# regicide211212/multi-style-transfer-gan

Measured on AMD Instinct MI355X. Metric: train-step images/sec (fwd+bwd+loss), 256x256 batch32, higher is better.
Workload: dtype f32; 1 GPU; config 3: reference CycleGAN train_step (2x EnhancedGenerator + 2x EnhancedDiscriminator, channels=16, num_transformer_blocks=0), 32 image pairs/GPU at 256x256, fwd+bwd+loss+Adam; per_gpu_batch=32, size=256, channels=16, parallelism=dp1, collective=none, losses_finite=True

## Files before the change

### multi-style-transfer-gan_amd/mstg_hip/csrc/common.h

```cpp
#pragma once
#include <hip/hip_runtime.h>
#include <stdint.h>
#include <stdio.h>
#include <string.h>

#include "mstg_hip.h"

typedef float f32x4 __attribute__((ext_vector_type(4)));
typedef float f32x2 __attribute__((ext_vector_type(2)));

namespace mstg {

extern thread_local char g_last_error[256];
inline int fail_launch(hipError_t e, const char* what) {
    snprintf(g_last_error, sizeof(g_last_error), "%s: %s", what, hipGetErrorString(e));
    return MSTG_E_LAUNCH;
}
inline int fail_arg(int code, const char* what) {
    snprintf(g_last_error, sizeof(g_last_error), "%s", what);
    return code;
}
#define MSTG_CHECK_LAUNCH(what)                                   \
    do {                                                          \
        hipError_t e__ = hipGetLastError();                       \
        if (e__ != hipSuccess) return mstg::fail_launch(e__, what); \
    } while (0)

extern bool g_prof_on;
void prof_begin(const void* host_fn, hipStream_t st);
void prof_end(hipStream_t st);
#define MSTG_LAUNCH(kern, grid, block, lds, st, ...)                               \
    do {                                                                           \
        const bool prof__ = mstg::g_prof_on;                                       \
        if (prof__) mstg::prof_begin((const void*)(kern), (hipStream_t)(st));      \
        hipLaunchKernelGGL(kern, grid, block, lds, st, __VA_ARGS__);               \
        if (prof__) mstg::prof_end((hipStream_t)(st));                             \
    } while (0)

extern thread_local bool t_ws_packed;
#define MSTG_PACK_LAUNCH(...)                      \
    do {                                           \
        if (!mstg::t_ws_packed) MSTG_LAUNCH(__VA_ARGS__); \
    } while (0)

enum EnvKnob {
    ENV_ATTN_BLK4, ENV_ATTN_BLK64, ENV_WGRAD_1X1, ENV_WGRAD_TS_MAXCH, ENV_WGRAD_PLAIN, ENV_WGRAD_OLD, ENV_NO_DPACK, ENV_IGEMM,
    ENV_STREAM, ENV_PF, ENV_WGLOB, ENV_HEAVY_PER_CU, ENV_DBG, ENV_DBG_LDS_KB, ENV_MS_WGRAD_PACKED, ENV_MS_FWD4, ENV_NO_PACK_CACHE,
    ENV_P32, ENV_P32_TH, ENV_P32_WLDS, ENV_P32_DBG, ENV_P32_OCC, ENV_ATTN_REG, ENV_NFW_ADAPT, ENV_BSUMS_ALL, ENV_ATTN_BIG32, ENV_NORM_WGS,
    ENV_CONV_IMG, ENV_COUNT
};
const char* env_get(EnvKnob k);

int cu_count();
struct OccCache {
    const void* kern = nullptr;
    size_t lds = 0;
    int occ = 1;
};
int persistent_occupancy(OccCache& c, const void* kern, size_t lds);

constexpr int WAVE = 64;

__device__ __forceinline__ f32x4 mfma16(float a, float b, f32x4 c) {
    return __builtin_amdgcn_mfma_f32_16x16x4f32(a, b, c, 0, 0, 0);
}

__device__ __forceinline__ float wave_sum(float v) {
#pragma unroll
    for (int o = 32; o > 0; o >>= 1) v += __shfl_xor(v, o, 64);
    return v;
}

__device__ __forceinline__ float apply_act(float v, int act) {
    switch (act) {
        case MSTG_ACT_RELU: return v > 0.f ? v : 0.f;
        case MSTG_ACT_LEAKY02: return v > 0.f ? v : 0.2f * v;
        case MSTG_ACT_TANH: return tanhf(v);
        case MSTG_ACT_GELU: return 0.5f * v * (1.f + erff(v * 0.70710678118654752f));
        default: return v;
    }
}
__device__ __forceinline__ float act_grad(float v, int act) {
    switch (act) {
        case MSTG_ACT_RELU: return v > 0.f ? 1.f : 0.f;
        case MSTG_ACT_LEAKY02: return v > 0.f ? 1.f : 0.2f;
        case MSTG_ACT_TANH: return 1.f - v * v;
        case MSTG_ACT_GELU: return 0.5f * (1.f + erff(v * 0.70710678118654752f)) + v * 0.3989422804014327f * expf(-0.5f * v * v);
        default: return 1.f;
    }
}

__device__ __forceinline__ int xcd_swizzle(int bid, int nblk) {
    const int q = nblk >> 3, r = nblk & 7, xcd = bid & 7, k = bid >> 3;
    return (xcd < r ? xcd * (q + 1) : r * (q + 1) + (xcd - r) * q) + k;
}


__host__ __device__ __forceinline__ unsigned magic_u32(unsigned d) { return 0xFFFFFFFFu / d + 1u; }

template <int NB>
__device__ __forceinline__ void stage_window_batch(const float* __restrict__ img, float* __restrict__ lds, int total, int e0, int cols,
                                                   int nq, unsigned m_cols, unsigned m_nq, int y0, int x0, int H, int W, int ctot,
                                                   int nq_valid, int ckp, int tid, int rowpad) {
    f32x4 v[NB];
    int dst[NB];
    bool ok[NB];
#pragma unroll
    for (int k = 0; k < NB; ++k) {
        const int e = e0 + 256 * k + tid;
        const int p = nq == 1 ? e : (int)__umulhi((unsigned)e, m_nq);
        const int q = e - p * nq;
        const int r = (int)__umulhi((unsigned)p, m_cols), c = p - r * cols;
        const int iy = y0 + r, ix = x0 + c;
        ok[k] = e < total && (unsigned)iy < (unsigned)H && (unsigned)ix < (unsigned)W && q < nq_valid;
        const unsigned off = ok[k] ? (unsigned)(iy * W + ix) * (unsigned)ctot + 4u * q : 0u;
        v[k] = *reinterpret_cast<const f32x4*>(img + off);
        dst[k] = e < total ? p * ckp + 4 * q + r * rowpad : -1;
    }
#pragma unroll
    for (int k = 0; k < NB; ++k)
        if (dst[k] >= 0) *reinterpret_cast<f32x4*>(&lds[dst[k]]) = ok[k] ? v[k] : f32x4{0.f, 0.f, 0.f, 0.f};
}

__device__ __forceinline__ void stage_window(const float* __restrict__ img, float* __restrict__ lds, int rows, int cols, int nq,
                                             unsigned m_cols, unsigned m_nq, int y0, int x0, int H, int W, int ctot, int nq_valid,
                                             int ckp, int tid, int rowpad = 0) {
    const int total = rows * cols * nq;
    int e0 = 0;
    for (; e0 + 1024 < total; e0 += 2048)
        stage_window_batch<8>(img, lds, total, e0, cols, nq, m_cols, m_nq, y0, x0, H, W, ctot, nq_valid, ckp, tid, rowpad);
    for (; e0 < total; e0 += 1024)
        stage_window_batch<4>(img, lds, total, e0, cols, nq, m_cols, m_nq, y0, x0, H, W, ctot, nq_valid, ckp, tid, rowpad);
// ... 38 lines not shown
```

### multi-style-transfer-gan_amd/mstg_hip/csrc/msblock.hip

```cpp
#include "common.h"
#include <stdlib.h>

namespace mstg {

constexpr int MS_TH = 8, MS_PH = MS_TH + 8, MS_PW = 16 + 8, MS_CKP = 20;

template <int CH>
__global__ __launch_bounds__(256) void wgrad_ms_kernel(const float* __restrict__ x, const float* __restrict__ dy,
                                                       float* __restrict__ partial, int N, int H, int W, int tiles_x, int tiles_y,
                                                       int ntiles) {
    constexpr int NFH = CH / 16, C4 = CH / 4, U = NFH + 24, UW = (U + 3) / 4, BNP = CH + 4, NG = CH / 16;
    constexpr int PSTRIDE = NG * U * 256 + CH;
    extern __shared__ __attribute__((aligned(16))) float smem[];
    float* patch = smem;
    float* ht = smem + MS_PH * MS_PW * MS_CKP;

    const int tid = threadIdx.x, lane = tid & 63, wave = tid >> 6, i = lane & 15, g = lane >> 4;
    const int gchunk = blockIdx.y, g0 = 16 * gchunk;

    f32x4 acc[UW];
    int toff[UW], hfo[UW];
#pragma unroll
    for (int k = 0; k < UW; ++k) {
        const int u = min(wave + 4 * k, U - 1);
        int dyp = 0, dxp = 0, frag = u;
        if (u >= NFH) {
            const int r = (u - NFH) >> 3, i8 = (u - NFH) & 7, t9 = i8 < 4 ? i8 : i8 + 1, d = 1 << r;
            dyp = (t9 / 3 - 1) * d;
            dxp = (t9 % 3 - 1) * d;
            frag = ((r + 1) * C4) / 16;
        }
        toff[k] = ((4 + dyp) * MS_PW + 4 + dxp) * MS_CKP;
        hfo[k] = 16 * frag;
        acc[k] = f32x4{0.f, 0.f, 0.f, 0.f};
    }
    const int nu = (U - wave + 3) / 4;

    const bool do_bias = gchunk == 0;
    float bsum = 0.f;
    const unsigned m_pw = magic_u32(MS_PW), m_nq = magic_u32(CH / 4);
    const size_t plane = (size_t)H * W;
    for (int tile = blockIdx.x; tile < ntiles; tile += gridDim.x) {
        const int tx0 = tile % tiles_x, ty0 = (tile / tiles_x) % tiles_y, n = tile / (tiles_x * tiles_y);
        __syncthreads();
        stage_window(x + (size_t)n * plane * CH + g0, patch, MS_PH, MS_PW, 4, m_pw, 0x40000000u, ty0 * MS_TH - 4, tx0 * 16 - 4, H, W, CH, 4,
                     MS_CKP, tid);
        stage_window(dy + (size_t)n * plane * CH, ht, MS_TH, 16, CH / 4, 0x10000000u, m_nq, ty0 * MS_TH, tx0 * 16, H, W, CH, CH / 4, BNP, tid);
        __syncthreads();
        if (do_bias && tid < CH) {
#pragma unroll 8
            for (int p = 0; p < MS_TH * 16; ++p) bsum += ht[p * BNP + tid];
        }
#pragma unroll 1
        for (int r = 0; r < MS_TH; ++r) {
#pragma unroll 2
            for (int xs = 0; xs < 4; ++xs) {
                const int c = 4 * xs + g;
                const int abase = (r * MS_PW + c) * MS_CKP + i;
                const int hbase = (r * 16 + c) * BNP + i;
                float af[UW], bf[UW];
#pragma unroll
                for (int k = 0; k < UW; ++k) { af[k] = patch[abase + toff[k]]; bf[k] = ht[hbase + hfo[k]]; }
#pragma unroll
                for (int k = 0; k < UW; ++k) acc[k] = mfma16(af[k], bf[k], acc[k]);
            }
        }
    }
    float* out = partial + (size_t)blockIdx.x * PSTRIDE;
    if (do_bias && tid < CH) out[NG * U * 256 + tid] = bsum;
#pragma unroll
    for (int k = 0; k < UW; ++k) {
        if (k >= nu) continue;
        const int u = wave + 4 * k;
        float* o = out + ((size_t)gchunk * U + u) * 256;
#pragma unroll
        for (int e = 0; e < 4; ++e) o[(4 * g + e) * 16 + i] = acc[k][e];
    }
}

template <int CH>
struct MsUnits {
    static constexpr int NFW = CH / 16, C4 = CH / 4, U = NFW + 24;
    __host__ __device__ static constexpr int ring(int u) { return (u - NFW) >> 3; }
    __host__ __device__ static constexpr int t9(int u) { return ((u - NFW) & 7) < 4 ? ((u - NFW) & 7) : ((u - NFW) & 7) + 1; }
    __host__ __device__ static constexpr int oy(int u) { return u < NFW ? 0 : (t9(u) / 3 - 1) * (1 << ring(u)); }
    __host__ __device__ static constexpr int ox(int u) { return u < NFW ? 0 : (t9(u) % 3 - 1) * (1 << ring(u)); }
    __host__ __device__ static constexpr int frag(int u) { return u < NFW ? u : ((ring(u) + 1) * C4) / 16; }
};

struct MsParamPtrs {
    const float* w[4];
    const float* b[4];
};

template <int CH>
__global__ void ms_pack_fwd_kernel(MsParamPtrs prm, float* __restrict__ wp) {
    typedef MsUnits<CH> G;
    constexpr int NCH = CH / 16, TOTAL = NCH * G::U * 256;
    for (int idx = blockIdx.x * blockDim.x + threadIdx.x; idx < TOTAL + CH; idx += gridDim.x * blockDim.x) {
        if (idx >= TOTAL) {
            const int co = idx - TOTAL;
            wp[idx] = prm.b[co / G::C4][co % G::C4];
            continue;
        }
        const int j = idx & 3, lane = (idx >> 2) & 63, u = (idx >> 8) % G::U, chunk = idx / (G::U * 256);
        const int i = lane & 15, g = lane >> 4, ci = 16 * chunk + 4 * g + j;
        float v = 0.f;
        if (u < G::NFW) {
            const int co = 16 * u + i, br = co / G::C4, cj = co % G::C4;
            v = br == 0 ? prm.w[0][cj * CH + ci] : prm.w[br][(cj * CH + ci) * 9 + 4];
        } else {
            const int r = (u - G::NFW) >> 3, i8 = (u - G::NFW) & 7, t9 = i8 < 4 ? i8 : i8 + 1, br = r + 1;
            const int co = 16 * ((br * G::C4) / 16) + i;
            if (co >= br * G::C4 && co < (br + 1) * G::C4) v = prm.w[br][((co - br * G::C4) * CH + ci) * 9 + t9];
        }
        wp[idx] = v;
    }
}

template <int CH, int UB, int UE>
struct MsFwdUnitLoop {
    template <typename ACC>
    static __device__ __forceinline__ void run(ACC& acc, const float* __restrict__ wpc, const float* __restrict__ patch, int pbase, int lane) {
        typedef MsUnits<CH> G;
        constexpr int u = UB;
        const f32x4 a = *reinterpret_cast<const f32x4*>(wpc + u * 256 + lane * 4);
        constexpr int off = (G::oy(u) * MS_PW + G::ox(u)) * MS_CKP;
        f32x4 b[2];
#pragma unroll
        for (int pf = 0; pf < 2; ++pf) b[pf] = *reinterpret_cast<const f32x4*>(&patch[pbase + pf * MS_PW * MS_CKP + off]);
#pragma unroll
        for (int j = 0; j < 4; ++j)
#pragma unroll
            for (int pf = 0; pf < 2; ++pf) acc[G::frag(u)][pf] = mfma16(a[j], b[pf][j], acc[G::frag(u)][pf]);
        MsFwdUnitLoop<CH, UB + 1, UE>::run(acc, wpc, patch, pbase, lane);
    }
};
template <int CH, int UE>
struct MsFwdUnitLoop<CH, UE, UE> {
    template <typename ACC>
    static __device__ __forceinline__ void run(ACC&, const float*, const float*, int, int) {}
};

template <int CH>
__global__ __launch_bounds__(256) void ms_fwd_kernel(const float* __restrict__ x, const float* __restrict__ wp, float* __restrict__ y,
                                                     int N, int H, int W, int tiles_x, int tiles_y) {
    typedef MsUnits<CH> G;
    constexpr int NFW = G::NFW, NCH = CH / 16, PF = 2;
    extern __shared__ __attribute__((aligned(16))) float smem[];
    float* patch = smem;
    const int tid = threadIdx.x, lane = tid & 63, wave = tid >> 6, i = lane & 15, g = lane >> 4;
    const int tile = xcd_swizzle(blockIdx.x, gridDim.x);
// ... 85 lines not shown
        for (int wf = 0; wf < NFW; ++wf) a[wf] = *reinterpret_cast<const f32x4*>(wpc + ((wf * K::NQ + Q) * 64 + lane) * 4);
#pragma unroll
        for (int e = 0; e < 4; ++e) {
            constexpr int s0 = 4 * Q;
            const int s = s0 + e;
            if (s < K::NS) {
                const int off = (K::oy(s) * MS_PW + K::ox(s)) * MS_CKP + 4 * K::grp(s);
                float b[2];
#pragma unroll
                for (int pf = 0; pf < 2; ++pf) b[pf] = patch[pbase + pf * MS_PW * MS_CKP + off];
#pragma unroll
                for (int wf = 0; wf < NFW; ++wf)
#pragma unroll
                    for (int pf = 0; pf < 2; ++pf) acc[wf][pf] = mfma16(a[wf][e], b[pf], acc[wf][pf]);
            }
        }
        MsDgQuadLoop<CH, C, QB + 1, QE>::run(acc, wpc, patch, pbase, lane);
    }
};
template <int CH, int C, int QE>
struct MsDgQuadLoop<CH, C, QE, QE> {
    template <typename ACC>
    static __device__ __forceinline__ void run(ACC&, const float*, const float*, int, int) {}
};

template <int CH, int C, typename ACC>
__device__ __forceinline__ void ms_dgrad_chunk(ACC& acc, const float* __restrict__ dy_img, const float* __restrict__ wp, float* patch,
                                               int ty0, int tx0, int H, int W, unsigned m_pw, int pbase, int tid, int lane) {
    typedef MsDgChunk<CH, C> K;
    constexpr int NFW = CH / 16;
    if (C) __syncthreads();
    stage_window(dy_img + 16 * C, patch, MS_PH, MS_PW, 4, m_pw, 0x40000000u, ty0 * MS_TH - 4, tx0 * 16 - 4, H, W, CH, 4, MS_CKP, tid);
    __syncthreads();
    MsDgQuadLoop<CH, C, 0, K::NQ>::run(acc, wp + (size_t)ms_dg_quads_before<CH>(C) * NFW * 256, patch, pbase, lane);
}

template <int CH>
__global__ __launch_bounds__(256) void ms_dgrad_kernel(const float* __restrict__ dy, const float* __restrict__ wp,
                                                       const float* __restrict__ dres, float* __restrict__ dx, int N, int H, int W,
                                                       int tiles_x, int tiles_y) {
    constexpr int NFW = CH / 16, PF = 2;
    extern __shared__ __attribute__((aligned(16))) float smem[];
    float* patch = smem;
    const int tid = threadIdx.x, lane = tid & 63, wave = tid >> 6, i = lane & 15, g = lane >> 4;
    const int tile = xcd_swizzle(blockIdx.x, gridDim.x);
    const int tx0 = tile % tiles_x, ty0 = (tile / tiles_x) % tiles_y, n = tile / (tiles_x * tiles_y);
    const size_t plane = (size_t)H * W;
    const unsigned m_pw = magic_u32(MS_PW);
    f32x4 acc[NFW][PF];
#pragma unroll
    for (int wf = 0; wf < NFW; ++wf)
#pragma unroll
        for (int pf = 0; pf < PF; ++pf) acc[wf][pf] = f32x4{0.f, 0.f, 0.f, 0.f};
    const int pbase = ((PF * wave + 4) * MS_PW + i + 4) * MS_CKP + g;
    const float* dy_img = dy + (size_t)n * plane * CH;
    ms_dgrad_chunk<CH, 0>(acc, dy_img, wp, patch, ty0, tx0, H, W, m_pw, pbase, tid, lane);
    if (CH >= 32) ms_dgrad_chunk<CH, (CH >= 32 ? 1 : 0)>(acc, dy_img, wp, patch, ty0, tx0, H, W, m_pw, pbase, tid, lane);
    if (CH >= 64) {
        ms_dgrad_chunk<CH, (CH >= 64 ? 2 : 0)>(acc, dy_img, wp, patch, ty0, tx0, H, W, m_pw, pbase, tid, lane);
        ms_dgrad_chunk<CH, (CH >= 64 ? 3 : 0)>(acc, dy_img, wp, patch, ty0, tx0, H, W, m_pw, pbase, tid, lane);
    }
#pragma unroll
    for (int pf = 0; pf < PF; ++pf) {
        const int gy = ty0 * MS_TH + PF * wave + pf, gx = tx0 * 16 + i;
        if (gy < H && gx < W) {
            const size_t o = (((size_t)n * H + gy) * W + gx) * CH + 4 * g;
#pragma unroll
            for (int wf = 0; wf < NFW; ++wf) {
                f32x4 v = acc[wf][pf];
                if (dres) v += *reinterpret_cast<const f32x4*>(dres + o + 16 * wf);
                *reinterpret_cast<f32x4*>(dx + o + 16 * wf) = v;
            }
        }
    }
}

template <int CH>
struct MsPk {
    static constexpr int NFH = CH / 16, C4 = CH / 4, TPU = 16 / C4, UPB = 8 / TPU, U = NFH + 3 * UPB, UW = (U + 3) / 4;
    static constexpr int NG = CH / 16, PSTRIDE = NG * U * 256 + CH, LDY = CH + 4;
};

template <int CH>
__global__ __launch_bounds__(256) void wgrad_msp_kernel(const float* __restrict__ x, const float* __restrict__ dy,
                                                        float* __restrict__ partial, int N, int H, int W, int tiles_x, int tiles_y,
                                                        int ntiles) {
    typedef MsPk<CH> G;
    constexpr int UW = G::UW, U = G::U, LDY = G::LDY, MG = G::NG, LDX = CH + 4;
    extern __shared__ __attribute__((aligned(16))) float smem[];
    float* xs = smem;
    float* dyp = smem + MS_TH * 16 * LDX;

    const int tid = threadIdx.x, lane = tid & 63, wave = tid >> 6, i = lane & 15, g = lane >> 4;

    f32x4 acc[UW][MG];
    int boff[UW];
#pragma unroll
    for (int k = 0; k < UW; ++k) {
        const int u = min(wave + 4 * k, U - 1);
        int off;
        if (u < G::NFH) {
            off = 16 * u + i;
        } else {
            const int j = 1 + (u - G::NFH) / G::UPB, m = (u - G::NFH) % G::UPB;
            const int sidx = i / G::C4, co = i % G::C4, i8 = m * G::TPU + sidx, t9 = i8 < 4 ? i8 : i8 + 1, d = 1 << (j - 1);
            const int oy = (t9 / 3 - 1) * d, ox = (t9 % 3 - 1) * d;
            off = (-oy * MS_PW - ox) * LDY + j * G::C4 + co;
        }
        boff[k] = off;
#pragma unroll
        for (int mf = 0; mf < MG; ++mf) acc[k][mf] = f32x4{0.f, 0.f, 0.f, 0.f};
    }
    const int nu = (U - wave + 3) / 4;

    float bsum = 0.f;
    const unsigned m_pw = magic_u32(MS_PW), m_nq = magic_u32(CH / 4);
    const size_t plane = (size_t)H * W;
    for (int tile = blockIdx.x; tile < ntiles; tile += gridDim.x) {
        const int tx0 = tile % tiles_x, ty0 = (tile / tiles_x) % tiles_y, n = tile / (tiles_x * tiles_y);
        __syncthreads();
        stage_window(x + (size_t)n * plane * CH, xs, MS_TH, 16, CH / 4, 0x10000000u, m_nq, ty0 * MS_TH, tx0 * 16, H, W, CH, CH / 4, LDX, tid);
        stage_window(dy + (size_t)n * plane * CH, dyp, MS_PH, MS_PW, CH / 4, m_pw, m_nq, ty0 * MS_TH - 4, tx0 * 16 - 4, H, W, CH, CH / 4, LDY,
                     tid);
        __syncthreads();
        if (tid < CH) {
            for (int r = 0; r < MS_TH; ++r)
#pragma unroll 8
                for (int c = 0; c < 16; ++c) bsum += dyp[((r + 4) * MS_PW + c + 4) * LDY + tid];
        }
#pragma unroll 1
        for (int r = 0; r < MS_TH; ++r) {
#pragma unroll 2
            for (int xs4 = 0; xs4 < 4; ++xs4) {
                const int c = 4 * xs4 + g;
                float af[MG], bf[UW];
#pragma unroll
                for (int mf = 0; mf < MG; ++mf) af[mf] = xs[(r * 16 + c) * LDX + 16 * mf + i];
                const int bbase = ((r + 4) * MS_PW + c + 4) * LDY;
#pragma unroll
                for (int k = 0; k < UW; ++k) bf[k] = dyp[bbase + boff[k]];
#pragma unroll
                for (int k = 0; k < UW; ++k)
#pragma unroll
                    for (int mf = 0; mf < MG; ++mf) acc[k][mf] = mfma16(af[mf], bf[k], acc[k][mf]);
            }
        }
    }
    float* out = partial + (size_t)blockIdx.x * G::PSTRIDE;
    if (tid < CH) out[G::NG * U * 256 + tid] = bsum;
#pragma unroll
    for (int k = 0; k < UW; ++k) {
        if (k >= nu) continue;
        const int u = wave + 4 * k;
#pragma unroll
        for (int mf = 0; mf < MG; ++mf) {
            float* o = out + ((size_t)mf * U + u) * 256;
#pragma unroll
            for (int e = 0; e < 4; ++e) o[(4 * g + e) * 16 + i] = acc[k][mf][e];
        }
    }
}

constexpr int M4_TH = 16, M4_PH = M4_TH + 8;

template <int CH, int JB, int T9, int Q>
struct Ms4Step {
    static constexpr int C4 = CH / 4, RS = C4 / 4;
    static __device__ __forceinline__ void run(f32x4 (&acc)[4][RS], const float* __restrict__ wl, const float* __restrict__ patch, int pbase,
                                               int wbase) {
        constexpr int d = JB == 0 ? 0 : (1 << (JB - 1));
        constexpr int oy = JB == 0 ? 0 : (T9 / 3 - 1) * d, ox = JB == 0 ? 0 : (T9 % 3 - 1) * d;
        constexpr int t = JB == 0 ? 0 : 1 + 9 * (JB - 1) + T9;
        const f32x4 b = *reinterpret_cast<const f32x4*>(&patch[pbase + (oy * MS_PW + ox) * MS_CKP + 4 * Q]);
#pragma unroll
        for (int rs = 0; rs < RS; ++rs) {
            const f32x4 a = *reinterpret_cast<const f32x4*>(&wl[wbase + (t * C4 + 4 * rs) * CH + 4 * Q]);
#pragma unroll
            for (int e = 0; e < 4; ++e) acc[JB][rs] = __builtin_amdgcn_mfma_f32_4x4x1f32(a[e], b[e], acc[JB][rs], 0, 0, 0);
        }
    }
};

template <int CH, int JB>
struct Ms4Branch {
    static constexpr int RS = CH / 16;
    static __device__ __forceinline__ void run(f32x4 (&acc)[4][RS], const float* wl, const float* patch, int pbase, int wbase) {
#define M4_TAP(T9)                                                  \
    Ms4Step<CH, JB, T9, 0>::run(acc, wl, patch, pbase, wbase);      \
    Ms4Step<CH, JB, T9, 1>::run(acc, wl, patch, pbase, wbase);      \
    Ms4Step<CH, JB, T9, 2>::run(acc, wl, patch, pbase, wbase);      \
    Ms4Step<CH, JB, T9, 3>::run(acc, wl, patch, pbase, wbase);
        if (JB == 0) {
            M4_TAP(0)
        } else {
            M4_TAP(0) M4_TAP(1) M4_TAP(2) M4_TAP(3) M4_TAP(4) M4_TAP(5) M4_TAP(6) M4_TAP(7) M4_TAP(8)
        }
#undef M4_TAP
    }
};

template <int CH>
__global__ __launch_bounds__(256) void ms_fwd4_kernel(const float* __restrict__ x, MsParamPtrs prm, float* __restrict__ y, int N, int H,
                                                      int W, int tiles_x, int tiles_y) {
    constexpr int C4 = CH / 4, RS = C4 / 4, NCHK = CH / 16;
    extern __shared__ __attribute__((aligned(16))) float smem[];
    float* patch = smem;
    float* wl = smem + M4_PH * MS_PW * MS_CKP;
    const int tid = threadIdx.x, lane = tid & 63, wave = tid >> 6;
    const int tile = xcd_swizzle(blockIdx.x, gridDim.x);
    const int tx0 = tile % tiles_x, ty0 = (tile / tiles_x) % tiles_y, n = tile / (tiles_x * tiles_y);
    const size_t plane = (size_t)H * W;
    for (int e = tid; e < 28 * C4 * CH; e += 256) {
        const int ci = e % CH, co = (e / CH) % C4, t = e / (CH * C4);
        float v;
        if (t == 0) v = prm.w[0][co * CH + ci];
        else v = prm.w[1 + (t - 1) / 9][(co * CH + ci) * 9 + (t - 1) % 9];
        wl[e] = v;
    }
    const int b = lane >> 2, j = lane & 3;
    const int prow = 4 * wave + (b >> 2), pcol = 4 * (b & 3) + j;
    const int pbase = ((prow + 4) * MS_PW + pcol + 4) * MS_CKP;
    f32x4 acc[4][RS];
#pragma unroll
    for (int jb = 0; jb < 4; ++jb)
#pragma unroll
        for (int rs = 0; rs < RS; ++rs) acc[jb][rs] = *reinterpret_cast<const f32x4*>(prm.b[jb] + 4 * rs);
    const unsigned m_pw = magic_u32(MS_PW);
#pragma unroll
    for (int chunk = 0; chunk < NCHK; ++chunk) {
        if (chunk) __syncthreads();
        stage_window(x + (size_t)n * plane * CH + 16 * chunk, patch, M4_PH, MS_PW, 4, m_pw, 0x40000000u, ty0 * M4_TH - 4, tx0 * 16 - 4, H, W,
                     CH, 4, MS_CKP, tid);
// ... 203 lines not shown
#pragma unroll
            for (int k = 0; k < 8; ++k) sum += v[k];
        }
        for (; sp < S; sp += 16) sum += partial[(size_t)sp * PSTRIDE + idx];
    }
    sh[row][e] = sum;
    __syncthreads();
    if (row != 0 || idx >= PSTRIDE) return;
    float r = 0.f;
#pragma unroll
    for (int k = 0; k < 16; ++k) r += sh[k][e];
    if (idx >= NACC) {
        const int co = idx - NACC;
        float* o = &out.db[co / C4][co % C4];
        *o = accumulate ? *o + r : r;
        return;
    }
    const int n = idx & 15, m = (idx >> 4) & 15, u = (idx >> 8) % U, gch = idx / (U * 256);
    const int ci = 16 * gch + m;
    if (u < NFH) {
        const int co = 16 * u + n, j = co / C4, cj = co % C4;
        float* o = j == 0 ? &out.dw[0][cj * CH + ci] : &out.dw[j][(cj * CH + ci) * 9 + 4];
        *o = accumulate ? *o + r : r;
    } else {
        const int rr = (u - NFH) >> 3, i8 = (u - NFH) & 7, t9 = i8 < 4 ? i8 : i8 + 1, j = rr + 1;
        const int co = 16 * ((j * C4) / 16) + n;
        if (co >= j * C4 && co < (j + 1) * C4) {
            float* o = &out.dw[j][((co - j * C4) * CH + ci) * 9 + t9];
            *o = accumulate ? *o + r : r;
        }
    }
}

template <int CH>
__global__ __launch_bounds__(256) void wgrad_msp_reduce_kernel(const float* __restrict__ partial, MsGradPtrs out, int S, int accumulate) {
    typedef MsPk<CH> G;
    constexpr int NACC = G::NG * G::U * 256, PSTRIDE = G::PSTRIDE, C4 = G::C4;
    __shared__ float sh[16][17];
    const int e = threadIdx.x & 15, row = threadIdx.x >> 4;
    const int idx = blockIdx.x * 16 + e;
    float sum = 0.f;
    if (idx < PSTRIDE) {
        int sp = row;
        for (; sp + 7 * 16 < S; sp += 8 * 16) {
            float v[8];
#pragma unroll
            for (int k = 0; k < 8; ++k) v[k] = partial[(size_t)(sp + 16 * k) * PSTRIDE + idx];
#pragma unroll
            for (int k = 0; k < 8; ++k) sum += v[k];
        }
        for (; sp < S; sp += 16) sum += partial[(size_t)sp * PSTRIDE + idx];
    }
    sh[row][e] = sum;
    __syncthreads();
    if (row != 0 || idx >= PSTRIDE) return;
    float r = 0.f;
#pragma unroll
    for (int k = 0; k < 16; ++k) r += sh[k][e];
    float* o;
    if (idx >= NACC) {
        const int co = idx - NACC;
        o = &out.db[co / C4][co % C4];
    } else {
        const int n = idx & 15, m = (idx >> 4) & 15, u = (idx >> 8) % G::U, gch = idx / (G::U * 256);
        const int ci = 16 * gch + m;
        if (u < G::NFH) {
            const int co = 16 * u + n, j = co / C4, cj = co % C4;
            o = j == 0 ? &out.dw[0][cj * CH + ci] : &out.dw[j][(cj * CH + ci) * 9 + 4];
        } else {
            const int j = 1 + (u - G::NFH) / G::UPB, mm = (u - G::NFH) % G::UPB;
            const int sidx = n / C4, co = n % C4, i8 = mm * G::TPU + sidx, t9 = i8 < 4 ? i8 : i8 + 1;
            o = &out.dw[j][(co * CH + ci) * 9 + t9];
        }
    }
    *o = accumulate ? *o + r : r;
}

template <int CH>
static bool ms_wgrad_packed() {
    const char* e = env_get(ENV_MS_WGRAD_PACKED);
    return CH <= 32 && !(e && e[0] == '0');
}

template <int CH>
static size_t ms_wgrad_plan(int N, int H, int W, int& S, int& tiles_x, int& tiles_y, int& ntiles) {
    constexpr int NFH = CH / 16, U = NFH + 24, NG = CH / 16, PSTRIDE = NG * U * 256 + CH;
    tiles_x = cdiv(W, 16);
    tiles_y = cdiv(H, MS_TH);
    ntiles = N * tiles_x * tiles_y;
    S = 768 / NG;
    if (S > ntiles) S = ntiles;
    if (S < 1) S = 1;
    size_t need = (size_t)S * PSTRIDE;
    if (CH <= 32) {
        const size_t sp = (size_t)S * NG > (size_t)ntiles ? (size_t)ntiles : (size_t)S * NG;
        const size_t np = sp * MsPk<(CH <= 32 ? CH : 16)>::PSTRIDE;
        if (np > need) need = np;
    }
    return need * sizeof(float);
}

template <int CH>
static int launch_ms_wgrad(const float* x, const float* dy, const MsGradPtrs& out, int accumulate, int N, int H, int W, void* ws,
                           size_t ws_bytes, hipStream_t st) {
    constexpr int NFH = CH / 16, U = NFH + 24, NG = CH / 16, PSTRIDE = NG * U * 256 + CH;
    int S, tiles_x, tiles_y, ntiles;
    const size_t need = ms_wgrad_plan<CH>(N, H, W, S, tiles_x, tiles_y, ntiles);
    if (!ws || ws_bytes < need) return fail_arg(MSTG_E_WORKSPACE, "msblock_wgrad: workspace too small");
    const size_t lds = (size_t)(MS_PH * MS_PW * MS_CKP + MS_TH * 16 * (CH + 4)) * sizeof(float);
    static bool attr_set = false;
    if (!attr_set) {
        hipError_t e = hipFuncSetAttribute(reinterpret_cast<const void*>(&wgrad_ms_kernel<CH>), hipFuncAttributeMaxDynamicSharedMemorySize,
                                           160 * 1024);
        if (e != hipSuccess) return fail_launch(e, "hipFuncSetAttribute(wgrad_ms)");
        attr_set = true;
    }
    if (ms_wgrad_packed<CH>()) {
        typedef MsPk<CH> P;
        const size_t ldsp = (size_t)(MS_TH * 16 * (CH + 4) + MS_PH * MS_PW * P::LDY) * sizeof(float);
        static bool attr_set_p = false;
        if (!attr_set_p) {
            hipError_t e = hipFuncSetAttribute(reinterpret_cast<const void*>(&wgrad_msp_kernel<CH>),
                                               hipFuncAttributeMaxDynamicSharedMemorySize, 160 * 1024);
            if (e != hipSuccess) return fail_launch(e, "hipFuncSetAttribute(wgrad_msp)");
            attr_set_p = true;
        }
        const int Sp = S * NG > ntiles ? ntiles : S * NG;
        MSTG_LAUNCH((wgrad_msp_kernel<CH>), dim3(Sp, 1, 1), dim3(256), ldsp, st, x, dy, (float*)ws, N, H, W, tiles_x, tiles_y, ntiles);
        MSTG_CHECK_LAUNCH("wgrad_msp_kernel");
        MSTG_LAUNCH((wgrad_msp_reduce_kernel<CH>), dim3(cdiv(P::PSTRIDE, 16)), dim3(256), 0, st, (const float*)ws, out, Sp, accumulate);
        MSTG_CHECK_LAUNCH("wgrad_msp_reduce_kernel");
        return MSTG_OK;
    }
    MSTG_LAUNCH((wgrad_ms_kernel<CH>), dim3(S, NG, 1), dim3(256), lds, st, x, dy, (float*)ws, N, H, W, tiles_x, tiles_y, ntiles);
    MSTG_CHECK_LAUNCH("wgrad_ms_kernel");
    MSTG_LAUNCH((wgrad_ms_reduce_kernel<CH>), dim3(cdiv(PSTRIDE, 16)), dim3(256), 0, st, (const float*)ws, out, S, accumulate);
    MSTG_CHECK_LAUNCH("wgrad_ms_reduce_kernel");
    return MSTG_OK;
}

template <int CH>
static int launch_ms_fwd(const float* x, const MsParamPtrs& prm, float* y, int N, int H, int W, void* ws, size_t ws_bytes, hipStream_t st) {
    typedef MsUnits<CH> G;
    {
        const char* e = env_get(ENV_MS_FWD4);
        bool aligned = true;
        for (int k = 0; k < 4; ++k) aligned = aligned && (reinterpret_cast<uintptr_t>(prm.b[k]) & 15) == 0;
        const bool use4b = CH <= 32 && (!e || e[0] == '3');
        const bool use4 = !use4b && ((CH == 16 && !(e && e[0] == '0')) || (CH == 32 && e && e[0] == '2'));
        if ((use4 || use4b) && aligned && H >= 16) {
            constexpr int C4K = (CH <= 32 ? CH : 16);
            const int tiles_x = cdiv(W, 16), tiles_y = cdiv(H, M4_TH);
            constexpr int LDW4B = C4K == 16 ? C4K : C4K + 4;
            const size_t lds = use4b ? (size_t)(M4_PH * M4B_ROW + 28 * (C4K / 4) * LDW4B) * sizeof(float)
                                     : (size_t)(M4_PH * MS_PW * MS_CKP + 28 * (C4K / 4) * C4K) * sizeof(float);
            static bool attr4 = false;
            if (!attr4) {
                hipError_t er = hipFuncSetAttribute(reinterpret_cast<const void*>(&ms_fwd4_kernel<C4K>),
                                                    hipFuncAttributeMaxDynamicSharedMemorySize, 160 * 1024);
                if (er == hipSuccess)
                    er = hipFuncSetAttribute(reinterpret_cast<const void*>(&ms_fwd4b_kernel<C4K>), hipFuncAttributeMaxDynamicSharedMemorySize,
                                             160 * 1024);
                if (er != hipSuccess) return fail_launch(er, "hipFuncSetAttribute(ms_fwd4)");
                attr4 = true;
            }
            if (use4b) {
                constexpr int PACKED = 28 * (C4K / 4) * LDW4B + C4K;
                if (!ws || ws_bytes < (size_t)PACKED * sizeof(float)) return fail_arg(MSTG_E_WORKSPACE, "msblock_fwd: workspace too small");
                MSTG_PACK_LAUNCH((ms_pack_fwd4b_kernel<C4K>), dim3(cdiv(PACKED, 256)), dim3(256), 0, st, prm, (float*)ws);
                MSTG_CHECK_LAUNCH("ms_pack_fwd4b_kernel");
                const int ntiles = N * tiles_x * tiles_y, slots = (C4K == 16 ? 3 : 2) * cu_count();
                MSTG_LAUNCH((ms_fwd4b_kernel<C4K>), dim3(ntiles < slots ? ntiles : slots), dim3(256), lds, st, x, (const float*)ws, y, N, H, W,
                            tiles_x, tiles_y, ntiles);
            } else MSTG_LAUNCH((ms_fwd4_kernel<C4K>), dim3(N * tiles_x * tiles_y), dim3(256), lds, st, x, prm, y, N, H, W, tiles_x, tiles_y);
            MSTG_CHECK_LAUNCH("ms_fwd4_kernel");
            return MSTG_OK;
        }
    }
    constexpr int NCH = CH / 16;
    const size_t need = (size_t)(NCH * G::U * 256 + CH) * sizeof(float);
    if (!ws || ws_bytes < need) return fail_arg(MSTG_E_WORKSPACE, "msblock_fwd: workspace too small");
    float* wp = (float*)ws;
    MSTG_PACK_LAUNCH((ms_pack_fwd_kernel<CH>), dim3(cdiv(NCH * G::U * 256 + CH, 256)), dim3(256), 0, st, prm, wp);
    MSTG_CHECK_LAUNCH("ms_pack_fwd_kernel");
    const int tiles_x = cdiv(W, 16), tiles_y = cdiv(H, MS_TH);
    const size_t lds = (size_t)(MS_PH * MS_PW * MS_CKP) * sizeof(float);
    MSTG_LAUNCH((ms_fwd_kernel<CH>), dim3(N * tiles_x * tiles_y), dim3(256), lds, st, x, (const float*)wp, y, N, H, W, tiles_x,
                       tiles_y);
    MSTG_CHECK_LAUNCH("ms_fwd_kernel");
    return MSTG_OK;
}

template <int CH>
static size_t ms_dgrad_ws_floats() {
    return (size_t)ms_dg_quads_before<CH>(CH / 16) * (CH / 16) * 256;
}

template <int CH>
static int launch_ms_dgrad(const float* dy, const MsParamPtrs& prm, const float* dres, float* dx, int N, int H, int W, void* ws,
                           size_t ws_bytes, hipStream_t st) {
    const size_t need = ms_dgrad_ws_floats<CH>() * sizeof(float);
    if (!ws || ws_bytes < need) return fail_arg(MSTG_E_WORKSPACE, "msblock_dgrad: workspace too small");
    float* wp = (float*)ws;
    MSTG_PACK_LAUNCH((ms_pack_dgrad_kernel<CH>), dim3(cdiv((int)ms_dgrad_ws_floats<CH>(), 1024)), dim3(256), 0, st, prm, wp);
    MSTG_CHECK_LAUNCH("ms_pack_dgrad_kernel");
    const int tiles_x = cdiv(W, 16), tiles_y = cdiv(H, MS_TH);
    const size_t lds = (size_t)(MS_PH * MS_PW * MS_CKP) * sizeof(float);
    MSTG_LAUNCH((ms_dgrad_kernel<CH>), dim3(N * tiles_x * tiles_y), dim3(256), lds, st, dy, (const float*)wp, dres, dx, N, H, W,
                       tiles_x, tiles_y);
    MSTG_CHECK_LAUNCH("ms_dgrad_kernel");
    return MSTG_OK;
}

}

using namespace mstg;
// ... 82 lines not shown
```

### multi-style-transfer-gan_amd/mstg_hip/csrc/runtime.hip

```cpp
#include <stdlib.h>

#include <cxxabi.h>

#include <mutex>
#include <string>
#include <vector>

#include "common.h"

namespace mstg {

thread_local char g_last_error[256] = "";
thread_local bool t_ws_packed = false;

static const char* const kEnvNames[ENV_COUNT] = {
    "MSTG_ATTN_BLK4", "MSTG_ATTN_BLK64", "MSTG_WGRAD_1X1", "MSTG_WGRAD_TS_MAXCH", "MSTG_WGRAD_PLAIN", "MSTG_WGRAD_OLD", "MSTG_NO_DPACK",
    "MSTG_IGEMM", "MSTG_STREAM", "MSTG_PF", "MSTG_WGLOB", "MSTG_HEAVY_PER_CU", "MSTG_DBG", "MSTG_DBG_LDS_KB", "MSTG_MS_WGRAD_PACKED",
    "MSTG_MS_FWD4", "MSTG_NO_PACK_CACHE", "MSTG_P32", "MSTG_P32_TH", "MSTG_P32_WLDS", "MSTG_P32_DBG", "MSTG_P32_OCC", "MSTG_ATTN_REG", "MSTG_NFW_ADAPT", "MSTG_BSUMS_ALL", "MSTG_ATTN_BIG32", "MSTG_NORM_WGS",
    "MSTG_CONV_IMG"};

struct EnvCache {
    char val[ENV_COUNT][32];
    bool set[ENV_COUNT];
    EnvCache() { refresh(); }
    void refresh() {
        for (int k = 0; k < ENV_COUNT; ++k) {
            const char* e = getenv(kEnvNames[k]);
            set[k] = e != nullptr;
            snprintf(val[k], sizeof(val[k]), "%s", e ? e : "");
        }
    }
};
static EnvCache g_env;

const char* env_get(EnvKnob k) { return g_env.set[k] ? g_env.val[k] : nullptr; }

int cu_count() {
    static int cus = 0;
    if (!cus) {
        int dev = 0;
        hipDeviceProp_t p;
        if (hipGetDevice(&dev) == hipSuccess && hipGetDeviceProperties(&p, dev) == hipSuccess) cus = p.multiProcessorCount;
        if (cus <= 0) cus = 256;
    }
    return cus;
}

int persistent_occupancy(OccCache& c, const void* kern, size_t lds) {
    if (c.kern != kern || c.lds != lds) {
        if (lds > 64 * 1024) (void)hipFuncSetAttribute(kern, hipFuncAttributeMaxDynamicSharedMemorySize, 160 * 1024);
        int nb = 1;
        if (hipOccupancyMaxActiveBlocksPerMultiprocessor(&nb, kern, 256, lds) != hipSuccess || nb < 1) nb = 1;
        c.occ = nb > 4 ? 4 : nb;
        c.kern = kern;
        c.lds = lds;
    }
    return c.occ;
}

bool g_prof_on = false;
struct ProfRec {
    const void* fn;
    hipStream_t st;
    hipEvent_t e0, e1;
};
static std::vector<ProfRec> g_prof;
static std::mutex g_prof_mu;
static thread_local int t_prof_open = -1;

void prof_begin(const void* fn, hipStream_t st) {
    ProfRec r{fn, st, nullptr, nullptr};
    if (hipEventCreate(&r.e0) != hipSuccess || hipEventCreate(&r.e1) != hipSuccess) return;
    (void)hipEventRecord(r.e0, st);
    std::lock_guard<std::mutex> lk(g_prof_mu);
    t_prof_open = (int)g_prof.size();
    g_prof.push_back(r);
}
void prof_end(hipStream_t st) {
    std::lock_guard<std::mutex> lk(g_prof_mu);
    if (t_prof_open < 0 || t_prof_open >= (int)g_prof.size()) return;
    (void)hipEventRecord(g_prof[t_prof_open].e1, st);
    t_prof_open = -1;
}
static void prof_clear() {
    for (auto& r : g_prof) {
        (void)hipEventDestroy(r.e0);
        (void)hipEventDestroy(r.e1);
    }
    g_prof.clear();
}

}

extern "C" const char* mstg_version(void) { return "mstg-hip 0.2.0 gfx950"; }
extern "C" const char* mstg_arch(void) { return "gfx950"; }
extern "C" const char* mstg_last_error(void) { return mstg::g_last_error; }
extern "C" void mstg_env_refresh(void) { mstg::g_env.refresh(); }

extern "C" int mstg_prof_enable(int on) {
    std::lock_guard<std::mutex> lk(mstg::g_prof_mu);
    if (on) mstg::prof_clear();
    mstg::g_prof_on = on != 0;
// ... 34 lines not shown
```

Measured before the change: 1728 images/sec.

## Prefetch next-tile windows into registers in multi-scale wgrad kernels and cap grid to occupancy

The multi-scale weight-gradient kernels now load the next tile's x and dy windows into registers while the current tile's MFMA loop runs, then commit them to LDS at the top of the next iteration. This hides global-load latency behind compute. The bias column sum is spread across all 256 threads and reduced through LDS at the end, replacing the previous 16-to-64-thread serial loop. Launch bounds now request multiple blocks per CU, and the persistent grid is capped at occupancy times CU count, with an env override. The prefetch registers raise VGPR pressure and could spill under the new launch-bound limits.

```diff
diff --git a/multi-style-transfer-gan_amd/mstg_hip/csrc/common.h b/multi-style-transfer-gan_amd/mstg_hip/csrc/common.h
--- a/multi-style-transfer-gan_amd/mstg_hip/csrc/common.h
+++ b/multi-style-transfer-gan_amd/mstg_hip/csrc/common.h
@@ -47,7 +47,7 @@
     ENV_ATTN_BLK4, ENV_ATTN_BLK64, ENV_WGRAD_1X1, ENV_WGRAD_TS_MAXCH, ENV_WGRAD_PLAIN, ENV_WGRAD_OLD, ENV_NO_DPACK, ENV_IGEMM,
     ENV_STREAM, ENV_PF, ENV_WGLOB, ENV_HEAVY_PER_CU, ENV_DBG, ENV_DBG_LDS_KB, ENV_MS_WGRAD_PACKED, ENV_MS_FWD4, ENV_NO_PACK_CACHE,
     ENV_P32, ENV_P32_TH, ENV_P32_WLDS, ENV_P32_DBG, ENV_P32_OCC, ENV_ATTN_REG, ENV_NFW_ADAPT, ENV_BSUMS_ALL, ENV_ATTN_BIG32, ENV_NORM_WGS,
-    ENV_CONV_IMG, ENV_COUNT
+    ENV_CONV_IMG, ENV_MS_WGRAD_WGS, ENV_COUNT
 };
 const char* env_get(EnvKnob k);
 
diff --git a/multi-style-transfer-gan_amd/mstg_hip/csrc/msblock.hip b/multi-style-transfer-gan_amd/mstg_hip/csrc/msblock.hip
--- a/multi-style-transfer-gan_amd/mstg_hip/csrc/msblock.hip
+++ b/multi-style-transfer-gan_amd/mstg_hip/csrc/msblock.hip
@@ -5,8 +5,39 @@
 
 constexpr int MS_TH = 8, MS_PH = MS_TH + 8, MS_PW = 16 + 8, MS_CKP = 20;
 
-template <int CH>
-__global__ __launch_bounds__(256) void wgrad_ms_kernel(const float* __restrict__ x, const float* __restrict__ dy,
+template <int NE>
+struct MsWinRegs {
+    f32x4 v[NE];
+    unsigned ok;
+};
+
+template <int NE, int ROWS, int COLS, int NQ>
+__device__ __forceinline__ void ms_win_fetch(MsWinRegs<NE>& R, const float* __restrict__ img, int y0, int x0, int H, int W, int ctot,
+                                             int tid) {
+    static_assert(ROWS * COLS * NQ == 256 * NE, "the window's quads divide evenly over the workgroup");
+    R.ok = 0;
+#pragma unroll
+    for (int k = 0; k < NE; ++k) {
+        const unsigned e = 256 * k + tid, p = e / NQ, q = e % NQ;
+        const int iy = y0 + (int)(p / COLS), ix = x0 + (int)(p % COLS);
+        const bool ok = (unsigned)iy < (unsigned)H && (unsigned)ix < (unsigned)W;
+        const unsigned off = ok ? (unsigned)(iy * W + ix) * (unsigned)ctot + 4u * q : 0u;
+        R.v[k] = *reinterpret_cast<const f32x4*>(img + off);
+        R.ok |= (unsigned)ok << k;
+    }
+}
+
+template <int NE, int NQ>
+__device__ __forceinline__ void ms_win_commit(const MsWinRegs<NE>& R, float* __restrict__ lds, int ckp, int tid) {
+#pragma unroll
+    for (int k = 0; k < NE; ++k) {
+        const unsigned e = 256 * k + tid;
+        *reinterpret_cast<f32x4*>(&lds[(e / NQ) * ckp + 4 * (e % NQ)]) = ((R.ok >> k) & 1) ? R.v[k] : f32x4{0.f, 0.f, 0.f, 0.f};
+    }
+}
+
+template <int CH>
+__global__ __launch_bounds__(256, CH == 64 ? 2 : 3) void wgrad_ms_kernel(const float* __restrict__ x, const float* __restrict__ dy,
                                                        float* __restrict__ partial, int N, int H, int W, int tiles_x, int tiles_y,
                                                        int ntiles) {
     constexpr int NFH = CH / 16, C4 = CH / 4, U = NFH + 24, UW = (U + 3) / 4, BNP = CH + 4, NG = CH / 16;
@@ -37,19 +68,28 @@
     const int nu = (U - wave + 3) / 4;
 
     const bool do_bias = gchunk == 0;
+    constexpr int BPARTS = 256 / CH;
+    const int bcol = tid % CH, bpart = tid / CH;
     float bsum = 0.f;
-    const unsigned m_pw = magic_u32(MS_PW), m_nq = magic_u32(CH / 4);
     const size_t plane = (size_t)H * W;
-    for (int tile = blockIdx.x; tile < ntiles; tile += gridDim.x) {
-        const int tx0 = tile % tiles_x, ty0 = (tile / tiles_x) % tiles_y, n = tile / (tiles_x * tiles_y);
+    constexpr int NX = MS_PH * MS_PW * 4 / 256, NY = MS_TH * 16 * (CH / 4) / 256;
+    MsWinRegs<NX> rx;
+    MsWinRegs<NY> ry;
+    auto fetch = [&](int t) {
+        const int tx0 = t % tiles_x, ty0 = (t / tiles_x) % tiles_y, n = t / (tiles_x * tiles_y);
+        ms_win_fetch<NX, MS_PH, MS_PW, 4>(rx, x + (size_t)n * plane * CH + g0, ty0 * MS_TH - 4, tx0 * 16 - 4, H, W, CH, tid);
+        ms_win_fetch<NY, MS_TH, 16, CH / 4>(ry, dy + (size_t)n * plane * CH, ty0 * MS_TH, tx0 * 16, H, W, CH, tid);
+    };
+    int tile = blockIdx.x;
+    if (tile < ntiles) fetch(tile);
+    for (; tile < ntiles; tile += gridDim.x) {
+        ms_win_commit<NX, 4>(rx, patch, MS_CKP, tid);
+        ms_win_commit<NY, CH / 4>(ry, ht, BNP, tid);
         __syncthreads();
-        stage_window(x + (size_t)n * plane * CH + g0, patch, MS_PH, MS_PW, 4, m_pw, 0x40000000u, ty0 * MS_TH - 4, tx0 * 16 - 4, H, W, CH, 4,
-                     MS_CKP, tid);
-        stage_window(dy + (size_t)n * plane * CH, ht, MS_TH, 16, CH / 4, 0x10000000u, m_nq, ty0 * MS_TH, tx0 * 16, H, W, CH, CH / 4, BNP, tid);
-        __syncthreads();
-        if (do_bias && tid < CH) {
-#pragma unroll 8
-            for (int p = 0; p < MS_TH * 16; ++p) bsum += ht[p * BNP + tid];
+        if (tile + (int)gridDim.x < ntiles) fetch(tile + gridDim.x);
+        if (do_bias) {
+#pragma unroll 4
+            for (int p = bpart; p < MS_TH * 16; p += BPARTS) bsum += ht[p * BNP + bcol];
         }
 #pragma unroll 1
         for (int r = 0; r < MS_TH; ++r) {
@@ -65,9 +105,19 @@
                 for (int k = 0; k < UW; ++k) acc[k] = mfma16(af[k], bf[k], acc[k]);
             }
         }
+        __syncthreads();
     }
     float* out = partial + (size_t)blockIdx.x * PSTRIDE;
-    if (do_bias && tid < CH) out[NG * U * 256 + tid] = bsum;
+    if (do_bias) {
+        smem[tid] = bsum;
+        __syncthreads();
+        if (tid < CH) {
+            bsum = 0.f;
+#pragma unroll
+            for (int j = 0; j < BPARTS; ++j) bsum += smem[tid + CH * j];
+            out[NG * U * 256 + tid] = bsum;
+        }
+    }
 #pragma unroll
     for (int k = 0; k < UW; ++k) {
         if (k >= nu) continue;
@@ -319,7 +369,7 @@
 };
 
 template <int CH>
-__global__ __launch_bounds__(256) void wgrad_msp_kernel(const float* __restrict__ x, const float* __restrict__ dy,
+__global__ __launch_bounds__(256, CH == 16 ? 3 : CH == 32 ? 2 : 1) void wgrad_msp_kernel(const float* __restrict__ x, const float* __restrict__ dy,
                                                         float* __restrict__ partial, int N, int H, int W, int tiles_x, int tiles_y,
                                                         int ntiles) {
     typedef MsPk<CH> G;
@@ -350,21 +400,27 @@
     }
     const int nu = (U - wave + 3) / 4;
 
+    constexpr int BPARTS = 256 / CH;
+    const int bcol = tid % CH, bpart = tid / CH;
     float bsum = 0.f;
-    const unsigned m_pw = magic_u32(MS_PW), m_nq = magic_u32(CH / 4);
     const size_t plane = (size_t)H * W;
-    for (int tile = blockIdx.x; tile < ntiles; tile += gridDim.x) {
-        const int tx0 = tile % tiles_x, ty0 = (tile / tiles_x) % tiles_y, n = tile / (tiles_x * tiles_y);
+    constexpr int NX = MS_TH * 16 * (CH / 4) / 256, NY = MS_PH * MS_PW * (CH / 4) / 256;
+    MsWinRegs<NX> rx;
+    MsWinRegs<NY> ry;
+    auto fetch = [&](int t) {
+        const int tx0 = t % tiles_x, ty0 = (t / tiles_x) % tiles_y, n = t / (tiles_x * tiles_y);
+        ms_win_fetch<NX, MS_TH, 16, CH / 4>(rx, x + (size_t)n * plane * CH, ty0 * MS_TH, tx0 * 16, H, W, CH, tid);
+        ms_win_fetch<NY, MS_PH, MS_PW, CH / 4>(ry, dy + (size_t)n * plane * CH, ty0 * MS_TH - 4, tx0 * 16 - 4, H, W, CH, tid);
+    };
+    int tile = blockIdx.x;
+    if (tile < ntiles) fetch(tile);
+    for (; tile < ntiles; tile += gridDim.x) {
+        ms_win_commit<NX, CH / 4>(rx, xs, LDX, tid);
+        ms_win_commit<NY, CH / 4>(ry, dyp, LDY, tid);
         __syncthreads();
-        stage_window(x + (size_t)n * plane * CH, xs, MS_TH, 16, CH / 4, 0x10000000u, m_nq, ty0 * MS_TH, tx0 * 16, H, W, CH, CH / 4, LDX, tid);
-        stage_window(dy + (size_t)n * plane * CH, dyp, MS_PH, MS_PW, CH / 4, m_pw, m_nq, ty0 * MS_TH - 4, tx0 * 16 - 4, H, W, CH, CH / 4, LDY,
-                     tid);
-        __syncthreads();
-        if (tid < CH) {
-            for (int r = 0; r < MS_TH; ++r)
-#pragma unroll 8
-                for (int c = 0; c < 16; ++c) bsum += dyp[((r + 4) * MS_PW + c + 4) * LDY + tid];
-        }
+        if (tile + (int)gridDim.x < ntiles) fetch(tile + gridDim.x);
+#pragma unroll 4
+        for (int p = bpart; p < MS_TH * 16; p += BPARTS) bsum += dyp[(((p >> 4) + 4) * MS_PW + (p & 15) + 4) * LDY + bcol];
 #pragma unroll 1
         for (int r = 0; r < MS_TH; ++r) {
 #pragma unroll 2
@@ -382,9 +438,17 @@
                     for (int mf = 0; mf < MG; ++mf) acc[k][mf] = mfma16(af[mf], bf[k], acc[k][mf]);
             }
         }
+        __syncthreads();
     }
     float* out = partial + (size_t)blockIdx.x * G::PSTRIDE;
-    if (tid < CH) out[G::NG * U * 256 + tid] = bsum;
+    smem[tid] = bsum;
+    __syncthreads();
+    if (tid < CH) {
+        bsum = 0.f;
+#pragma unroll
+        for (int j = 0; j < BPARTS; ++j) bsum += smem[tid + CH * j];
+        out[G::NG * U * 256 + tid] = bsum;
+    }
 #pragma unroll
     for (int k = 0; k < UW; ++k) {
         if (k >= nu) continue;
@@ -754,13 +818,22 @@
     return CH <= 32 && !(e && e[0] == '0');
 }
 
+constexpr int MS_WGRAD_MAX_WGS = 768;
+static int ms_wgrad_slots(OccCache& occ, const void* kern, size_t lds) {
+    int slots = persistent_occupancy(occ, kern, lds) * cu_count();
+    if (slots > MS_WGRAD_MAX_WGS) slots = MS_WGRAD_MAX_WGS;
+    const char* e = env_get(ENV_MS_WGRAD_WGS);
+    if (e && atoi(e) >= 1 && atoi(e) < slots) slots = atoi(e);
+    return slots;
+}
+
 template <int CH>
 static size_t ms_wgrad_plan(int N, int H, int W, int& S, int& tiles_x, int& tiles_y, int& ntiles) {
     constexpr int NFH = CH / 16, U = NFH + 24, NG = CH / 16, PSTRIDE = NG * U * 256 + CH;
     tiles_x = cdiv(W, 16);
     tiles_y = cdiv(H, MS_TH);
     ntiles = N * tiles_x * tiles_y;
-    S = 768 / NG;
+    S = MS_WGRAD_MAX_WGS / NG;
     if (S > ntiles) S = ntiles;
     if (S < 1) S = 1;
     size_t need = (size_t)S * PSTRIDE;
@@ -797,13 +870,19 @@
             if (e != hipSuccess) return fail_launch(e, "hipFuncSetAttribute(wgrad_msp)");
             attr_set_p = true;
         }
-        const int Sp = S * NG > ntiles ? ntiles : S * NG;
+        static OccCache occ_p;
+        int Sp = S * NG > ntiles ? ntiles : S * NG;
+        const int slots = ms_wgrad_slots(occ_p, reinterpret_cast<const void*>(&wgrad_msp_kernel<CH>), ldsp);
+        if (Sp > slots) Sp = slots;
         MSTG_LAUNCH((wgrad_msp_kernel<CH>), dim3(Sp, 1, 1), dim3(256), ldsp, st, x, dy, (float*)ws, N, H, W, tiles_x, tiles_y, ntiles);
         MSTG_CHECK_LAUNCH("wgrad_msp_kernel");
         MSTG_LAUNCH((wgrad_msp_reduce_kernel<CH>), dim3(cdiv(P::PSTRIDE, 16)), dim3(256), 0, st, (const float*)ws, out, Sp, accumulate);
         MSTG_CHECK_LAUNCH("wgrad_msp_reduce_kernel");
         return MSTG_OK;
     }
+    static OccCache occ_u;
+    const int Su = ms_wgrad_slots(occ_u, reinterpret_cast<const void*>(&wgrad_ms_kernel<CH>), lds) / NG;
+    if (S > Su) S = Su < 1 ? 1 : Su;
     MSTG_LAUNCH((wgrad_ms_kernel<CH>), dim3(S, NG, 1), dim3(256), lds, st, x, dy, (float*)ws, N, H, W, tiles_x, tiles_y, ntiles);
     MSTG_CHECK_LAUNCH("wgrad_ms_kernel");
     MSTG_LAUNCH((wgrad_ms_reduce_kernel<CH>), dim3(cdiv(PSTRIDE, 16)), dim3(256), 0, st, (const float*)ws, out, S, accumulate);
diff --git a/multi-style-transfer-gan_amd/mstg_hip/csrc/runtime.hip b/multi-style-transfer-gan_amd/mstg_hip/csrc/runtime.hip
--- a/multi-style-transfer-gan_amd/mstg_hip/csrc/runtime.hip
+++ b/multi-style-transfer-gan_amd/mstg_hip/csrc/runtime.hip
@@ -17,7 +17,7 @@
     "MSTG_ATTN_BLK4", "MSTG_ATTN_BLK64", "MSTG_WGRAD_1X1", "MSTG_WGRAD_TS_MAXCH", "MSTG_WGRAD_PLAIN", "MSTG_WGRAD_OLD", "MSTG_NO_DPACK",
     "MSTG_IGEMM", "MSTG_STREAM", "MSTG_PF", "MSTG_WGLOB", "MSTG_HEAVY_PER_CU", "MSTG_DBG", "MSTG_DBG_LDS_KB", "MSTG_MS_WGRAD_PACKED",
     "MSTG_MS_FWD4", "MSTG_NO_PACK_CACHE", "MSTG_P32", "MSTG_P32_TH", "MSTG_P32_WLDS", "MSTG_P32_DBG", "MSTG_P32_OCC", "MSTG_ATTN_REG", "MSTG_NFW_ADAPT", "MSTG_BSUMS_ALL", "MSTG_ATTN_BIG32", "MSTG_NORM_WGS",
-    "MSTG_CONV_IMG"};
+    "MSTG_CONV_IMG", "MSTG_MS_WGRAD_WGS"};
 
 struct EnvCache {
     char val[ENV_COUNT][32];
```

Result: no change. 1739 images/sec (median of 6 runs) (+0.7%).
